# PKU-Alignment/SafeVLA

Hardware: AMD Instinct MI355X
Metric: env-steps/sec through PPO-Lagrangian update (higher is better)
Workload: dtype bf16

## Files before the change

### safevla_amd/csrc/attn.hip

```cpp
#include "common.h"
#include "attn_hd96.h"
#include "attn_long.h"

#ifndef ATT_SWZ_OLD
#define ATT_SWZ_OLD 0
#endif
#ifndef ATT_EARLY_TR
#define ATT_EARLY_TR 0
#endif
#define HD 64
#define LDSROW 64
#define ATT_THREADS 256

enum { MASK_NONE = 0, MASK_BLOCK_CAUSAL = 1 };

struct AttnArgs {
    const bf16_t *Q, *K, *V; long ld;
    bf16_t* O; long ldo;
    float* LSE;
    const bf16_t* dO; long lddo;
    bf16_t *dQ, *dK, *dV; long ldd;
    const int* traj;
    const float* bias;
    const unsigned char* kvalid;
    int S, H, mask_mode;
    float scale;
    int kv_rows;
    int Sq;
    long ldq, lddq;
    float* Dws;
    DropCfg drop;
    int xcd_rows;
};

__device__ __forceinline__ unsigned long long att_drop_row(const AttnArgs& p, int r, int h, int q) {
    return ((unsigned long long)((size_t)r * p.H + h) * p.S + q) * (unsigned long long)((p.S + 3) & ~3);
}
__device__ __forceinline__ bool att_keep1(const DropCfg& c, unsigned long long e) {
    const unsigned x = drop_bits(c.key, e >> 1);
    return ((e & 1) ? (x >> 16) : (x & 0xffffu)) >= c.thr;
}

__device__ __forceinline__ int att_swz(int row) {
    const int x = (row >> 1) & 7;
    return ATT_SWZ_OLD ? x : ((((x + ((x >> 2) << 1)) & 3) << 1) | (x >> 2));
}

struct RowBase { const bf16_t* lo; const bf16_t* hi; };
__device__ __forceinline__ RowBase att_row_base(const bf16_t* tile, int lane) {
    const int ql = lane & 15, g = lane >> 4, f = att_swz(ql);
    return RowBase{tile + ql * LDSROW + ((g ^ f) << 3), tile + ql * LDSROW + (((g + 4) ^ f) << 3)};
}
struct TrBase { const bf16_t* d[4]; };
__device__ __forceinline__ TrBase att_tr_base(const bf16_t* tile, int lane) {
    const int ql = lane & 15, g = lane >> 4;
    const int row = 4 * g + (ql >> 2), f = att_swz(row);
    TrBase t;
#pragma unroll
    for (int dt = 0; dt < 4; ++dt) t.d[dt] = tile + row * LDSROW + (((2 * dt + ((ql & 3) >> 1)) ^ f) << 3) + 4 * (ql & 1);
    return t;
}
__device__ __forceinline__ bf16x8 lds_row8i(const bf16_t* lane_base, int tile_row0) {
    return *(const bf16x8*)(lane_base + tile_row0 * LDSROW);
}
__device__ __forceinline__ bf16x8 lds_tr8i(const bf16_t* lane_base_dt, int rA, int rB) {
    const bf16x4 lo = lds_tr16_b64(lane_base_dt + rA * LDSROW);
    const bf16x4 hi = lds_tr16_b64(lane_base_dt + rB * LDSROW);
    return bf16x8{lo[0], lo[1], lo[2], lo[3], hi[0], hi[1], hi[2], hi[3]};
}
__device__ __forceinline__ bf16x8 pack8(const float (&v)[8]) {
    u32x4 w;
#pragma unroll
    for (int i = 0; i < 4; ++i) w[i] = pack_bf2(v[2 * i], v[2 * i + 1]);
    return __builtin_bit_cast(bf16x8, w);
}
#define LOG2E 1.4426950408889634f
#define LN2 0.6931471805599453f

template <int SP, int THREADS = ATT_THREADS>
__device__ __forceinline__ void stage_head(bf16_t* dst, const bf16_t* src, long ld, int S, int tid) {
    constexpr int IT = SP * 8 / THREADS;
    u32x4 w[IT];
#pragma unroll
    for (int i = 0; i < IT; ++i) {
        const int q = tid + i * THREADS;
        const int row = q >> 3, c = q & 7;
        w[i] = u32x4{0, 0, 0, 0};
        if (row < S) w[i] = *(const u32x4*)(src + (size_t)row * ld + c * 8);
    }
#pragma unroll
    for (int i = 0; i < IT; ++i) {
        const int q = tid + i * THREADS;
        *(u32x4*)(dst + (q >> 3) * LDSROW + (((q & 7) ^ att_swz(q >> 3)) << 3)) = w[i];
    }
}

__device__ __forceinline__ bool masked(const AttnArgs& p, int q, int key, const int* traj_s, const unsigned char* kv_s) {
    if (key >= p.S) return true;
    if (p.mask_mode == MASK_BLOCK_CAUSAL && (key > q || traj_s[key] != traj_s[q])) return true;
    if (kv_s && !kv_s[key]) return true;
    return false;
}

template <int NKT, bool GENERIC, int NW = 4, bool EXACT = false>
__device__ __forceinline__ void attn_fwd_kernel_body(AttnArgs p) {
    p.drop = drop_resolve(p.drop);
    extern __shared__ __attribute__((aligned(16))) char smem[];
    constexpr int SP = NKT * 16;
    bf16_t* Ks = (bf16_t*)smem;
    bf16_t* Vs = Ks + SP * LDSROW;
    int* traj_s = (int*)(Vs + SP * LDSROW);
    unsigned char* kv_s = (unsigned char*)(traj_s + SP);
    const int tid = threadIdx.x, lane = tid & 63, wid = tid >> 6;
    const int r = blockIdx.x / p.H, h = blockIdx.x % p.H;
    const size_t tok0 = (size_t)r * p.kv_rows, mtok0 = (size_t)r * p.S;
    const int S = p.S;
    stage_head<SP, NW * 64>(Ks, p.K + tok0 * p.ld + h * HD, p.ld, S, tid);
    stage_head<SP, NW * 64>(Vs, p.V + tok0 * p.ld + h * HD, p.ld, S, tid);
    for (int i = tid; i < SP; i += NW * 64) {
        traj_s[i] = (p.traj && i < S) ? p.traj[mtok0 + i] : -1;
        kv_s[i] = (p.kvalid && i < S) ? p.kvalid[mtok0 + i] : 1;
    }
    const int ql = lane & 15, g = lane >> 4;
    const int Sq = p.Sq;
    const size_t qtok0 = (size_t)r * Sq;
    const int nqt = (Sq + 15) / 16;
    constexpr int MAXQT = (NKT + NW - 1) / NW;
    bf16x8 qall[MAXQT][2];
#pragma unroll
    for (int t = 0; t < MAXQT; ++t) {
        const int q = (wid + NW * t) * 16 + ql;
        const bool ok = q < Sq;
        const bf16_t* qp = p.Q + (qtok0 + (ok ? q : 0)) * p.ldq + h * HD + 8 * g;
        qall[t][0] = ok ? *(const bf16x8*)qp : bf16x8{0, 0, 0, 0, 0, 0, 0, 0};
        qall[t][1] = ok ? *(const bf16x8*)(qp + 32) : bf16x8{0, 0, 0, 0, 0, 0, 0, 0};
    }
    __syncthreads();
    const unsigned char* kvp = p.kvalid ? kv_s : nullptr;
    const RowBase Krow = att_row_base(Ks, lane);
    const TrBase Vtr = att_tr_base(Vs, lane);
#pragma unroll
    for (int t = 0; t < MAXQT; ++t) {
        const int qt = wid + NW * t;
        if (qt >= nqt) break;
        const int q = qt * 16 + ql;
        const bf16x8 qf[2] = {qall[t][0], qall[t][1]};
        float sc[NKT][4];
        float mx = -INFINITY;
        const float sl2 = p.scale * LOG2E;
#pragma unroll
        for (int kt = 0; kt < NKT; ++kt) {
            f32x4 a = {0.f, 0.f, 0.f, 0.f};
            if (EXACT || kt * 16 < S) {
                a = mfma16(lds_row8i(Krow.lo, kt * 16), qf[0], a);
                a = mfma16(lds_row8i(Krow.hi, kt * 16), qf[1], a);
            }
            if constexpr (GENERIC) {
#pragma unroll
                for (int e = 0; e < 4; ++e) {
                    const int key = kt * 16 + 4 * g + e;
                    float s = a[e] * p.scale;
                    if (p.bias && q < Sq && key < S) s += p.bias[((size_t)h * S + q) * S + key];
                    s *= LOG2E;
                    if (masked(p, q < Sq ? q : 0, key, traj_s, kvp)) s = -INFINITY;
                    sc[kt][e] = s;
                    mx = fmaxf(mx, s);
                }
            } else {
                const bool tail = EXACT ? kt >= NKT - 2 : (kt + 1) * 16 > S;
#pragma unroll
                for (int e = 0; e < 4; ++e) {
                    float s = a[e] * sl2;
                    if (tail && kt * 16 + 4 * g + e >= S) s = -INFINITY;
                    sc[kt][e] = s;
                    mx = fmaxf(mx, s);
                }
            }
        }
        mx = fmaxf(mx, __shfl_xor(mx, 16, 64));
        mx = fmaxf(mx, __shfl_xor(mx, 32, 64));
        if (mx == -INFINITY) mx = 0.f;
        float lsum = 0.f;
#pragma unroll
        for (int kt = 0; kt < NKT; ++kt)
#pragma unroll
            for (int e = 0; e < 4; ++e) { sc[kt][e] = __builtin_amdgcn_exp2f(sc[kt][e] - mx); lsum += sc[kt][e]; }
        lsum += __shfl_xor(lsum, 16, 64);
        lsum += __shfl_xor(lsum, 32, 64);
        if (p.drop.thr) {
            const unsigned long long rb = att_drop_row(p, r, h, q < Sq ? q : 0);
#pragma unroll
            for (int kt = 0; kt < NKT; ++kt) {
                const unsigned keep = drop_keep4(p.drop, rb + kt * 16 + 4 * g);
#pragma unroll
                for (int e = 0; e < 4; ++e) if (!((keep >> e) & 1u)) sc[kt][e] = 0.f;
            }
        }
        f32x4 o[4];
#pragma unroll
        for (int dt = 0; dt < 4; ++dt) o[dt] = f32x4{0.f, 0.f, 0.f, 0.f};
#pragma unroll
        for (int u = 0; u < NKT / 2; ++u) {
            if (EXACT || u * 32 < S) {
                const float pv[8] = {sc[2 * u][0], sc[2 * u][1], sc[2 * u][2], sc[2 * u][3],
                                     sc[2 * u + 1][0], sc[2 * u + 1][1], sc[2 * u + 1][2], sc[2 * u + 1][3]};
                const bf16x8 pa = pack8(pv);
#pragma unroll
                for (int dt = 0; dt < 4; ++dt)
                    o[dt] = mfma16(lds_tr8i(Vtr.d[dt], 32 * u, 32 * u + 16), pa, o[dt]);
            }
        }
        const float inv = lsum > 0.f ? p.drop.scale / lsum : 0.f;
        if (q < Sq) {
#pragma unroll
            for (int dt = 0; dt < 4; ++dt) {
                const u32x2 w = {pack_bf2(o[dt][0] * inv, o[dt][1] * inv), pack_bf2(o[dt][2] * inv, o[dt][3] * inv)};
                *(u32x2*)(p.O + (qtok0 + q) * p.ldo + h * HD + dt * 16 + 4 * g) = w;
            }
        }
        if (p.LSE && g == 0 && q < Sq) p.LSE[((size_t)r * p.H + h) * Sq + q] = (mx + __log2f(lsum)) * LN2;
    }
}

__device__ __forceinline__ void att_xcd_item(const AttnArgs& p, int item, int nitems, int& r, int& h) {
    if (!p.xcd_rows) return;
    const int x = item & 7, j = item >> 3, nfull = (nitems / 64) * 8;
    if ((j >> 3) * 8 + x < nfull) { r = (j >> 3) * 8 + x; h = j & 7; }
}
struct AttDrop {
    unsigned a0;
    unsigned hb;
    bool wrap;
    unsigned long long p0;
};
__device__ __forceinline__ AttDrop att_drop_head(const AttnArgs& p, int r, int h) {
    AttDrop d;
    d.p0 = att_drop_row(p, r, h, 0) >> 1;
    d.a0 = (unsigned)d.p0 * 0x9E3779B1u;
    d.hb = ((unsigned)(d.p0 >> 32) * 0x85EBCA77u) ^ p.drop.key;
    d.wrap = (unsigned)d.p0 > 0xFFFF0000u;
    return d;
}

template <int NKT>
__device__ __forceinline__ void attn_fwd_persist_kernel_body(AttnArgs p, int nitems) {
    p.drop = drop_resolve(p.drop);
    extern __shared__ __attribute__((aligned(16))) char smem[];
    constexpr int SP = NKT * 16, IT = SP * 8 / ATT_THREADS, MAXQT = (NKT + 3) / 4;
    bf16_t* Ks = (bf16_t*)smem;
    bf16_t* Vs = Ks + SP * LDSROW;
    const int tid = threadIdx.x, lane = tid & 63, wid = tid >> 6;
    const int ql = lane & 15, g = lane >> 4;
    const int S = p.S, Sq = p.Sq, nqt = (Sq + 15) / 16;
    u32x4 kreg[IT], vreg[IT];
    bf16x8 qreg[MAXQT][2];
    auto fetch = [&](int item) {
        int r = item / p.H, h = item % p.H;
        att_xcd_item(p, item, nitems, r, h);
        const bf16_t* kp = p.K + (size_t)r * p.kv_rows * p.ld + h * HD;
        const bf16_t* vp = p.V + (size_t)r * p.kv_rows * p.ld + h * HD;
#pragma unroll
        for (int i = 0; i < IT; ++i) {
            const int q = tid + i * ATT_THREADS, row = q >> 3, c = q & 7;
            kreg[i] = u32x4{0, 0, 0, 0}; vreg[i] = u32x4{0, 0, 0, 0};
            if (row < S) {
                kreg[i] = *(const u32x4*)(kp + (size_t)row * p.ld + c * 8);
                vreg[i] = *(const u32x4*)(vp + (size_t)row * p.ld + c * 8);
            }
        }
#pragma unroll
        for (int t = 0; t < MAXQT; ++t) {
            const int q = (wid + 4 * t) * 16 + ql;
            const bool ok = q < Sq;
            const bf16_t* qp = p.Q + ((size_t)r * Sq + (ok ? q : 0)) * p.ldq + h * HD + 8 * g;
            qreg[t][0] = ok ? *(const bf16x8*)qp : bf16x8{0, 0, 0, 0, 0, 0, 0, 0};
            qreg[t][1] = ok ? *(const bf16x8*)(qp + 32) : bf16x8{0, 0, 0, 0, 0, 0, 0, 0};
        }
    };
    int item = blockIdx.x;
    if (item >= nitems) return;
    fetch(item);
    const RowBase Krow = att_row_base(Ks, lane);
    const TrBase Vtr = att_tr_base(Vs, lane);
    const float sl2 = p.scale * LOG2E;
    for (; item < nitems; item += gridDim.x) {
        int r = item / p.H, h = item % p.H;
        att_xcd_item(p, item, nitems, r, h);
        const size_t qtok0 = (size_t)r * Sq;
        __syncthreads();
#pragma unroll
        for (int i = 0; i < IT; ++i) {
            const int q = tid + i * ATT_THREADS;
            const int off = (q >> 3) * LDSROW + (((q & 7) ^ att_swz(q >> 3)) << 3);
            *(u32x4*)(Ks + off) = kreg[i];
            *(u32x4*)(Vs + off) = vreg[i];
        }
        bf16x8 qcur[MAXQT][2];
#pragma unroll
        for (int t = 0; t < MAXQT; ++t) { qcur[t][0] = qreg[t][0]; qcur[t][1] = qreg[t][1]; }
        __syncthreads();
        if (item + (int)gridDim.x < nitems) fetch(item + gridDim.x);
#pragma unroll
        for (int t = 0; t < MAXQT; ++t) {
            const int qt = wid + 4 * t;
// ... 508 lines not shown
#pragma unroll
                for (int dt = 0; dt < 4; ++dt) {
                    const u32x2 wk = {pack_bf2(dk[dt][0], dk[dt][1]), pack_bf2(dk[dt][2], dk[dt][3])};
                    const u32x2 wv = {pack_bf2(dv[dt][0], dv[dt][1]), pack_bf2(dv[dt][2], dv[dt][3])};
                    *(u32x2*)(p.dK + (tok0 + keyl) * p.ldd + h * HD + dt * 16 + 4 * g) = wk;
                    *(u32x2*)(p.dV + (tok0 + keyl) * p.ldd + h * HD + dt * 16 + 4 * g) = wv;
                }
            }
        }
    }
}

__device__ __forceinline__ f32x4 fma4(f32x4 a, f32x4 b, f32x4 c) { return __builtin_elementwise_fma(a, b, c); }

template <int NKT, bool DROP>
__global__ void __launch_bounds__(ATT_THREADS, NKT <= 12 ? 3 : 2) attn_bwd_fused_exact_kernel(AttnArgs p) {
    if (DROP) p.drop = drop_resolve(p.drop);
#ifdef ATT_TIMING
    const long long tm0 = __builtin_readcyclecounter();
#endif
    extern __shared__ __attribute__((aligned(16))) char smem[];
    constexpr int SP = NKT * 16, MAXT = (NKT + 3) / 4, IT = SP * 8 / ATT_THREADS;
    constexpr bool EARLY_TR = ATT_EARLY_TR && NKT <= 12;
    constexpr bool KEEP_KV = true;
    bf16_t* As = (bf16_t*)smem;
    bf16_t* Bs = As + SP * LDSROW;
    float* nl_s = (float*)(Bs + SP * LDSROW);
    float* nd_s = nl_s + SP;
    const int tid = threadIdx.x, lane = tid & 63, wid = tid >> 6;
    int r = blockIdx.x / p.H, h = blockIdx.x % p.H;
    att_xcd_item(p, blockIdx.x, gridDim.x, r, h);
    const size_t tok0 = (size_t)r * p.S, qtok0 = (size_t)r * p.Sq;
    const int S = p.S, Sq = p.Sq;
    const int ql = lane & 15, g = lane >> 4;
    constexpr int NBUF = KEEP_KV ? MAXT : 2;
    bf16x8 kvbuf[NBUF][4];
    auto load_kv = [&](int t, bf16x8 (&dst)[4]) {
        const int keyl = (wid + 4 * t) * 16 + ql;
        const bool kok = keyl < S;
        const bf16_t* kp = p.K + (tok0 + (kok ? keyl : 0)) * p.ld + h * HD + 8 * g;
        const bf16_t* vp = p.V + (tok0 + (kok ? keyl : 0)) * p.ld + h * HD + 8 * g;
        dst[0] = gld8(kp, kok); dst[1] = gld8(kp + 32, kok);
        dst[2] = gld8(vp, kok); dst[3] = gld8(vp + 32, kok);
    };
    load_kv(0, kvbuf[0]);
    if (KEEP_KV) {
#pragma unroll
        for (int t = 1; t < MAXT; ++t) if (wid + 4 * t < NKT) load_kv(t, kvbuf[t]);
    }
    stage_head<SP>(As, p.Q + qtok0 * p.ldq + h * HD, p.ldq, Sq, tid);
    {
        u32x4 w[IT];
        float part[IT];
#pragma unroll
        for (int i = 0; i < IT; ++i) {
            const int q = tid + i * ATT_THREADS, row = q >> 3, c = q & 7;
            const bool ok = row < Sq;
            const bf16x8 gv = gld8(p.dO + (qtok0 + (ok ? row : 0)) * p.lddo + h * HD + c * 8, ok);
            const bf16x8 ov = gld8(p.O + (qtok0 + (ok ? row : 0)) * p.ldo + h * HD + c * 8, ok);
            w[i] = __builtin_bit_cast(u32x4, gv);
            part[i] = dot8(gv, ov);
        }
#pragma unroll
        for (int i = 0; i < IT; ++i) {
            const int q = tid + i * ATT_THREADS, row = q >> 3;
            *(u32x4*)(Bs + row * LDSROW + (((q & 7) ^ att_swz(row)) << 3)) = w[i];
            float d = part[i];
            d += __shfl_xor(d, 1, 64); d += __shfl_xor(d, 2, 64); d += __shfl_xor(d, 4, 64);
            if ((q & 7) == 0) nd_s[row] = -d * p.scale;
        }
    }
    for (int i = tid; i < SP; i += ATT_THREADS)
        nl_s[i] = i < Sq ? -p.LSE[((size_t)r * p.H + h) * Sq + i] * LOG2E : -INFINITY;
    __syncthreads();
#ifdef ATT_TIMING
    const long long tm1 = __builtin_readcyclecounter();
#endif
    const float sl2 = p.scale * LOG2E;
    const float dsc = DROP ? p.drop.scale : 1.f, scd = p.scale * dsc;
    const f32x4 sl4 = {sl2, sl2, sl2, sl2}, scd4 = {scd, scd, scd, scd}, dsc4 = {dsc, dsc, dsc, dsc};
    const RowBase Arow = att_row_base(As, lane), Brow = att_row_base(Bs, lane);
    const TrBase Atr = att_tr_base(As, lane), Btr = att_tr_base(Bs, lane);
    const int S4 = (S + 3) & ~3, hS = S4 >> 1;
    AttDrop dh{};
    if (DROP) dh = att_drop_head(p, r, h);
    const unsigned thr = p.drop.thr;
    {
        const int nw = (Sq + 31) / 32;
        const int odd = ql & 1;
        const unsigned dl_a = (unsigned)((4 * g + 2 * odd) * hS + (ql >> 1));
        const unsigned al_a = dh.a0 + dl_a * 0x9E3779B1u;
        const unsigned hSC = (unsigned)hS * 0x9E3779B1u;
#pragma unroll
        for (int t = 0; t < MAXT; ++t) {
            const int kt = wid + 4 * t;
            __builtin_amdgcn_sched_barrier(0);
            if (kt < NKT) {
                const int keyl = kt * 16 + ql;
                const bool kok = keyl < S;
                if (!KEEP_KV && t + 1 < MAXT && kt + 4 < NKT) load_kv(t + 1, kvbuf[(t + 1) % NBUF]);
                const bf16x8 kf0 = kvbuf[t % NBUF][0], kf1 = kvbuf[t % NBUF][1], vf0 = kvbuf[t % NBUF][2], vf1 = kvbuf[t % NBUF][3];
                f32x4 dk[4], dv[4];
#pragma unroll
                for (int dt = 0; dt < 4; ++dt) { dk[dt] = f32x4{0.f, 0.f, 0.f, 0.f}; dv[dt] = f32x4{0.f, 0.f, 0.f, 0.f}; }
#pragma unroll (NKT <= 12 ? 2 : 1)
                for (int w = 0; w < nw; ++w) {
                    const int off = w * 32 * LDSROW;
                    float pv[8], dsv[8];
                    bf16x8 gfr[4], qfr[4];
                    if (EARLY_TR) {
#pragma unroll
                        for (int dt = 0; dt < 4; ++dt) { gfr[dt] = lds_tr8i(Btr.d[dt] + off, 0, 16); qfr[dt] = lds_tr8i(Atr.d[dt] + off, 0, 16); }
                    }
#pragma unroll
                    for (int e2 = 0; e2 < 2; ++e2) {
                        const int o2 = off + e2 * 16 * LDSROW;
                        f32x4 sv = {0.f, 0.f, 0.f, 0.f}, dp = {0.f, 0.f, 0.f, 0.f};
                        sv = mfma16(*(const bf16x8*)(Arow.lo + o2), kf0, sv);
                        sv = mfma16(*(const bf16x8*)(Arow.hi + o2), kf1, sv);
                        dp = mfma16(*(const bf16x8*)(Brow.lo + o2), vf0, dp);
                        dp = mfma16(*(const bf16x8*)(Brow.hi + o2), vf1, dp);
                        const f32x4 nl4 = *(const f32x4*)(nl_s + w * 32 + e2 * 16 + 4 * g), nd4 = *(const f32x4*)(nd_s + w * 32 + e2 * 16 + 4 * g);
                        const f32x4 x = fma4(sv, sl4, nl4);
                        f32x4 pr;
#pragma unroll
                        for (int e = 0; e < 4; ++e) pr[e] = __builtin_amdgcn_exp2f(x[e]);
                        f32x4 pd = pr, tt = fma4(dp, scd4, nd4);
                        if (DROP) {
                            pd = pr * dsc4;
                            unsigned keep;
                            if (!dh.wrap) {
                                const int qb = w * 32 + e2 * 16;
                                const unsigned ua = (unsigned)(qb * hS + kt * 8) * 0x9E3779B1u;
                                const unsigned x0 = drop_mix((al_a + ua) ^ dh.hb), x1 = drop_mix((al_a + ua + hSC) ^ dh.hb);
                                const unsigned mine = odd ? ((x0 >> 16) | (x1 & 0xffff0000u)) : ((x0 & 0xffffu) | (x1 << 16));
                                const unsigned give = odd ? ((x0 & 0xffffu) | (x1 << 16)) : ((x0 >> 16) | (x1 & 0xffff0000u));
                                const unsigned got = (unsigned)__builtin_amdgcn_mov_dpp((int)give, 0xB1, 0xf, 0xf, true);
                                const unsigned q01 = odd ? got : mine, q23 = odd ? mine : got;
                                keep = ((q01 & 0xffffu) >= thr ? 1u : 0u) | ((q01 >> 16) >= thr ? 2u : 0u) | ((q23 & 0xffffu) >= thr ? 4u : 0u) | ((q23 >> 16) >= thr ? 8u : 0u);
                            } else {
                                keep = 0;
#pragma unroll
                                for (int e = 0; e < 4; ++e) {
                                    const int q = w * 32 + e2 * 16 + 4 * g + e;
                                    keep |= att_keep1(p.drop, (dh.p0 << 1) + (unsigned)(q * S4 + keyl)) ? (1u << e) : 0u;
                                }
                            }
#pragma unroll
                            for (int e = 0; e < 4; ++e) {
                                const bool kp = (keep >> e) & 1u;
                                pd[e] = kp ? pd[e] : 0.f;
                                tt[e] = kp ? tt[e] : nd4[e];
                            }
                        }
                        const f32x4 ds = pr * tt;
#pragma unroll
                        for (int e = 0; e < 4; ++e) { pv[e2 * 4 + e] = pd[e]; dsv[e2 * 4 + e] = ds[e]; }
                    }
                    const bf16x8 pa = pack8(pv), da = pack8(dsv);
#pragma unroll
                    for (int dt = 0; dt < 4; ++dt) {
                        if (!EARLY_TR) { gfr[dt] = lds_tr8i(Btr.d[dt] + off, 0, 16); qfr[dt] = lds_tr8i(Atr.d[dt] + off, 0, 16); }
                        dv[dt] = mfma16(gfr[dt], pa, dv[dt]);
                        dk[dt] = mfma16(qfr[dt], da, dk[dt]);
                    }
                }
                if (kok) {
#pragma unroll
                    for (int dt = 0; dt < 4; ++dt) {
                        const u32x2 wk = {pack_bf2(dk[dt][0], dk[dt][1]), pack_bf2(dk[dt][2], dk[dt][3])};
                        const u32x2 wv = {pack_bf2(dv[dt][0], dv[dt][1]), pack_bf2(dv[dt][2], dv[dt][3])};
                        *(u32x2*)(p.dK + (tok0 + keyl) * p.ldd + h * HD + dt * 16 + 4 * g) = wk;
                        *(u32x2*)(p.dV + (tok0 + keyl) * p.ldd + h * HD + dt * 16 + 4 * g) = wv;
                    }
                }
            }
        }
    }
    __builtin_amdgcn_sched_barrier(0);
#ifdef ATT_TIMING
    const long long tm2 = __builtin_readcyclecounter();
#endif
    bf16x8 qall[MAXT][4];
    float dall[MAXT], lall[MAXT];
#pragma unroll
    for (int t = 0; t < MAXT; ++t) {
        const int qt = wid + 4 * t;
        if (qt < NKT) {
            const int o = qt * 16 * LDSROW;
            qall[t][0] = *(const bf16x8*)(Arow.lo + o); qall[t][1] = *(const bf16x8*)(Arow.hi + o);
            qall[t][2] = *(const bf16x8*)(Brow.lo + o); qall[t][3] = *(const bf16x8*)(Brow.hi + o);
            lall[t] = nl_s[qt * 16 + ql]; dall[t] = nd_s[qt * 16 + ql];
        }
    }
    __syncthreads();
    if (KEEP_KV) {
        const int f = att_swz(ql);
#pragma unroll
        for (int t = 0; t < MAXT; ++t) {
            const int kt = wid + 4 * t;
            if (kt < NKT) {
                bf16_t* ka = As + (kt * 16 + ql) * LDSROW;
                bf16_t* va = Bs + (kt * 16 + ql) * LDSROW;
                *(bf16x8*)(ka + ((g ^ f) << 3)) = kvbuf[t % NBUF][0]; *(bf16x8*)(ka + (((g + 4) ^ f) << 3)) = kvbuf[t % NBUF][1];
                *(bf16x8*)(va + ((g ^ f) << 3)) = kvbuf[t % NBUF][2]; *(bf16x8*)(va + (((g + 4) ^ f) << 3)) = kvbuf[t % NBUF][3];
            }
        }
    } else {
        stage_head<SP>(As, p.K + tok0 * p.ld + h * HD, p.ld, S, tid);
        stage_head<SP>(Bs, p.V + tok0 * p.ld + h * HD, p.ld, S, tid);
    }
    __syncthreads();
#ifdef ATT_TIMING
    const long long tm3 = __builtin_readcyclecounter();
#endif
    {
        const int ntile = (Sq + 15) / 16;
        const unsigned dl_b = (unsigned)(ql * hS + 2 * g);
        const unsigned al_b = dh.a0 + dl_b * 0x9E3779B1u;
#pragma unroll
        for (int t = 0; t < MAXT; ++t) {
            const int qt = wid + 4 * t;
            __builtin_amdgcn_sched_barrier(0);
            if (qt < ntile) {
                const int q = qt * 16 + ql;
                const bool qok = q < Sq;
                const f32x4 nl4 = {lall[t], lall[t], lall[t], lall[t]}, nd4 = {dall[t], dall[t], dall[t], dall[t]};
                f32x4 dq[4];
#pragma unroll
                for (int dt = 0; dt < 4; ++dt) dq[dt] = f32x4{0.f, 0.f, 0.f, 0.f};
#pragma unroll (NKT <= 12 ? 2 : 1)
                for (int u = 0; u < NKT / 2; ++u) {
                    const int off = u * 32 * LDSROW;
                    float dsv[8];
#pragma unroll
                    for (int e2 = 0; e2 < 2; ++e2) {
                        const int o2 = off + e2 * 16 * LDSROW;
                        f32x4 sv = {0.f, 0.f, 0.f, 0.f}, dp = {0.f, 0.f, 0.f, 0.f};
                        sv = mfma16(*(const bf16x8*)(Arow.lo + o2), qall[t][0], sv);
                        sv = mfma16(*(const bf16x8*)(Arow.hi + o2), qall[t][1], sv);
                        dp = mfma16(*(const bf16x8*)(Brow.lo + o2), qall[t][2], dp);
                        dp = mfma16(*(const bf16x8*)(Brow.hi + o2), qall[t][3], dp);
                        const f32x4 x = fma4(sv, sl4, nl4);
                        f32x4 pr;
#pragma unroll
                        for (int e = 0; e < 4; ++e) pr[e] = __builtin_amdgcn_exp2f(x[e]);
                        f32x4 tt = fma4(dp, scd4, nd4);
                        if (DROP) {
                            unsigned keep;
                            if (!dh.wrap) {
                                const unsigned ub = (unsigned)(qt * 16 * hS + (2 * u + e2) * 8) * 0x9E3779B1u;
                                const unsigned r0 = drop_mix((al_b + ub) ^ dh.hb), r1 = drop_mix((al_b + ub + 0x9E3779B1u) ^ dh.hb);
                                keep = ((r0 & 0xffffu) >= thr ? 1u : 0u) | ((r0 >> 16) >= thr ? 2u : 0u) | ((r1 & 0xffffu) >= thr ? 4u : 0u) | ((r1 >> 16) >= thr ? 8u : 0u);
                            } else {
                                keep = drop_keep4(p.drop, (dh.p0 << 1) + (unsigned long long)(qok ? q : 0) * S4 + (2 * u + e2) * 16 + 4 * g);
                            }
#pragma unroll
                            for (int e = 0; e < 4; ++e) tt[e] = ((keep >> e) & 1u) ? tt[e] : nd4[e];
                        }
                        const f32x4 ds = pr * tt;
#pragma unroll
                        for (int e = 0; e < 4; ++e) dsv[e2 * 4 + e] = ds[e];
                    }
                    const bf16x8 da = pack8(dsv);
#pragma unroll
                    for (int dt = 0; dt < 4; ++dt)
                        dq[dt] = mfma16(lds_tr8i(Atr.d[dt] + off, 0, 16), da, dq[dt]);
                }
                if (qok) {
#pragma unroll
                    for (int dt = 0; dt < 4; ++dt) {
                        const u32x2 w = {pack_bf2(dq[dt][0], dq[dt][1]), pack_bf2(dq[dt][2], dq[dt][3])};
                        *(u32x2*)(p.dQ + (qtok0 + q) * p.lddq + h * HD + dt * 16 + 4 * g) = w;
                    }
                }
            }
        }
    }
#ifdef ATT_TIMING
    if (p.kvalid && lane == 0) {
        __builtin_amdgcn_sched_barrier(0);
        const long long tm4 = __builtin_readcyclecounter();
        unsigned* d = (unsigned*)p.kvalid + ((size_t)blockIdx.x * 4 + wid) * 4;
        d[0] = (unsigned)(tm1 - tm0); d[1] = (unsigned)(tm2 - tm1); d[2] = (unsigned)(tm3 - tm2); d[3] = (unsigned)(tm4 - tm3);
    }
#endif
}

template <int NKT>
static int launch_fwd(const AttnArgs& p, int rows, hipStream_t st) {
    const size_t lds = (size_t)2 * NKT * 16 * LDSROW * sizeof(bf16_t) + NKT * 16 * (sizeof(int) + 1);
    const bool generic = p.mask_mode != MASK_NONE || p.bias || p.kvalid;
    if constexpr (NKT == 12 || NKT == 16) {
        if (!generic && p.S > (NKT - 2) * 16) {
            const size_t ldsp = (size_t)2 * NKT * 16 * LDSROW * sizeof(bf16_t);
            static int slots = 0;
            if (!slots) {
                int dev = 0, n_cu = 0;
                HIP_CHECK_RET(hipGetDevice(&dev));
                HIP_CHECK_RET(hipDeviceGetAttribute(&n_cu, hipDeviceAttributeMultiprocessorCount, dev));
                slots = 2 * n_cu;
            }
            const int nitems = rows * p.H;
            const int gslots = (slots / svla_group_size()) & ~7;
            return SVLA_LAUNCH_TWIN((attn_fwd_persist_kernel_body<NKT>), ATT_THREADS, 2, dim3(nitems < gslots ? nitems : gslots), dim3(ATT_THREADS), ldsp, st, p, nitems);
        }
    }
    if constexpr (NKT == 18) {
        if (!generic && p.S > (NKT - 2) * 16 && p.Sq == p.S)
            return SVLA_LAUNCH_TWIN((attn_fwd_kernel_body<NKT, false, 4, true>), ATT_THREADS, 1, dim3(rows * p.H), dim3(ATT_THREADS), lds, st, p);
    }
    if constexpr (NKT >= 28) {
        if (!generic) {
            if (p.S > (NKT - 2) * 16 && p.Sq == p.S) return SVLA_LAUNCH_TWIN((attn_fwd_kernel_body<NKT, false, 8, true>), 512, 1, dim3(rows * p.H), dim3(512), lds, st, p);
            return SVLA_LAUNCH_TWIN((attn_fwd_kernel_body<NKT, false, 8>), 512, 1, dim3(rows * p.H), dim3(512), lds, st, p);
        }
    }
    if (generic) return SVLA_LAUNCH_TWIN((attn_fwd_kernel_body<NKT, true>), ATT_THREADS, 1, dim3(rows * p.H), dim3(ATT_THREADS), lds, st, p);
    return SVLA_LAUNCH_TWIN((attn_fwd_kernel_body<NKT, false>), ATT_THREADS, 1, dim3(rows * p.H), dim3(ATT_THREADS), lds, st, p);
}
static int g_attn_no_decode = 0;
static int g_attn_bwd_two_pass = 0;
static int g_attn_xcd_rows = 1;
extern "C" int svla_attn_bwd_two_pass(int on) { g_attn_bwd_two_pass = on & 1; g_attn_xcd_rows = !(on & 2); g_attn_no_decode = (on & 4) ? 1 : 0; return 0; }

template <int NKT>
static int launch_bwd(const AttnArgs& p, int rows, hipStream_t st) {
    const size_t lds_q = (size_t)2 * NKT * 16 * LDSROW * sizeof(bf16_t) + NKT * 16 * (sizeof(int) + 1);
    const size_t lds_kv = (size_t)2 * NKT * 16 * LDSROW * sizeof(bf16_t) + NKT * 16 * (2 * sizeof(float) + sizeof(int) + 1);
    static bool attr = false;
    if (!attr) {
        HIP_CHECK_RET(hipFuncSetAttribute((const void*)attn_bwd_dq_kernel<NKT, true>, hipFuncAttributeMaxDynamicSharedMemorySize, (int)lds_q));
        HIP_CHECK_RET(hipFuncSetAttribute((const void*)attn_bwd_dkv_kernel<NKT, true>, hipFuncAttributeMaxDynamicSharedMemorySize, (int)lds_kv));
        HIP_CHECK_RET(hipFuncSetAttribute((const void*)attn_bwd_dq_kernel<NKT, false>, hipFuncAttributeMaxDynamicSharedMemorySize, (int)lds_q));
        HIP_CHECK_RET(hipFuncSetAttribute((const void*)attn_bwd_dkv_kernel<NKT, false>, hipFuncAttributeMaxDynamicSharedMemorySize, (int)lds_kv));
        attr = true;
    }
    const bool generic = p.mask_mode != MASK_NONE || p.bias || p.kvalid;
    if constexpr (NKT <= 16) if (!generic && (p.Dws || !g_attn_bwd_two_pass) && p.S > (NKT - 3) * 16) {
        const size_t le_q = (size_t)2 * NKT * 16 * LDSROW * sizeof(bf16_t);
        const size_t le_kv = le_q + NKT * 16 * 2 * sizeof(float);
        static bool attr_e = false;
        if (!attr_e) {
            HIP_CHECK_RET(hipFuncSetAttribute((const void*)attn_bwd_dq_exact_kernel<NKT>, hipFuncAttributeMaxDynamicSharedMemorySize, (int)le_q));
            HIP_CHECK_RET(hipFuncSetAttribute((const void*)attn_bwd_dkv_exact_kernel<NKT>, hipFuncAttributeMaxDynamicSharedMemorySize, (int)le_kv));
            HIP_CHECK_RET(hipFuncSetAttribute((const void*)attn_bwd_fused_exact_kernel<NKT, true>, hipFuncAttributeMaxDynamicSharedMemorySize, (int)le_kv));
            HIP_CHECK_RET(hipFuncSetAttribute((const void*)attn_bwd_fused_exact_kernel<NKT, false>, hipFuncAttributeMaxDynamicSharedMemorySize, (int)le_kv));
            attr_e = true;
        }
        if (g_attn_bwd_two_pass) {
            hipLaunchKernelGGL((attn_bwd_dq_exact_kernel<NKT>), dim3(rows * p.H), dim3(ATT_THREADS), le_q, st, p);
            hipLaunchKernelGGL((attn_bwd_dkv_exact_kernel<NKT>), dim3(rows * p.H), dim3(ATT_THREADS), le_kv, st, p);
        } else {
#ifdef ATT_TIMING
            AttnArgs pt = p; if (getenv("SVLA_ATTN_DBGBUF")) pt.kvalid = (const unsigned char*)strtoull(getenv("SVLA_ATTN_DBGBUF"), nullptr, 16);
            if (p.drop.thr) { hipLaunchKernelGGL((attn_bwd_fused_exact_kernel<NKT, true>), dim3(rows * p.H), dim3(ATT_THREADS), le_kv, st, pt); return svla_launch_status(); }
#endif
            if (p.drop.thr) hipLaunchKernelGGL((attn_bwd_fused_exact_kernel<NKT, true>), dim3(rows * p.H), dim3(ATT_THREADS), le_kv, st, p);
            else hipLaunchKernelGGL((attn_bwd_fused_exact_kernel<NKT, false>), dim3(rows * p.H), dim3(ATT_THREADS), le_kv, st, p);
        }
        return svla_launch_status();
    }
    if (generic) {
        hipLaunchKernelGGL((attn_bwd_dq_kernel<NKT, true>), dim3(rows * p.H), dim3(ATT_THREADS), lds_q, st, p);
        hipLaunchKernelGGL((attn_bwd_dkv_kernel<NKT, true>), dim3(rows * p.H), dim3(ATT_THREADS), lds_kv, st, p);
    } else {
        hipLaunchKernelGGL((attn_bwd_dq_kernel<NKT, false>), dim3(rows * p.H), dim3(ATT_THREADS), lds_q, st, p);
        hipLaunchKernelGGL((attn_bwd_dkv_kernel<NKT, false>), dim3(rows * p.H), dim3(ATT_THREADS), lds_kv, st, p);
    }
    return svla_launch_status();
}

#define DEC_THREADS 256
#define DEC_MAXB 16
__device__ __forceinline__ void attn_decode_kernel_body(AttnArgs p) {
    __shared__ float red[4][2];
    __shared__ float accs[4][64];
    const int tid = threadIdx.x, lane = tid & 63, wid = tid >> 6;
    const int g = tid >> 3, c = tid & 7;
    const int r = blockIdx.x / p.H, h = blockIdx.x % p.H;
    const int S = p.S;
    const size_t tok0 = (size_t)r * p.kv_rows;
    const unsigned char* kvr = p.kvalid ? p.kvalid + (size_t)r * S : nullptr;
    const float sl2 = p.scale * LOG2E;
    float qv[8];
    {
        const bf16x8 q8 = *(const bf16x8*)(p.Q + (size_t)r * p.ldq + h * HD + c * 8);
#pragma unroll
        for (int e = 0; e < 8; ++e) qv[e] = bf2f((bf16_t)q8[e]);
    }
    const int nb = (S + 31) >> 5;
    float sc[DEC_MAXB];
    unsigned vmask = 0;
    float mx = -INFINITY;
#pragma unroll
    for (int b = 0; b < DEC_MAXB; ++b) {
        sc[b] = -INFINITY;
        if (b < nb) {
            const int key = b * 32 + g;
            const bool ok = key < S && (!kvr || kvr[key]);
            if (ok) {
                const bf16x8 k8 = *(const bf16x8*)(p.K + (tok0 + key) * p.ld + h * HD + c * 8);
                float d = 0.f;
#pragma unroll
                for (int e = 0; e < 8; ++e) d = fmaf(qv[e], bf2f((bf16_t)k8[e]), d);
                sc[b] = d;
                vmask |= 1u << b;
            }
            float d = ok ? sc[b] : 0.f;
            d += __shfl_xor(d, 1, 64); d += __shfl_xor(d, 2, 64); d += __shfl_xor(d, 4, 64);
            sc[b] = ok ? d * sl2 : -INFINITY;
            mx = fmaxf(mx, sc[b]);
        }
    }
    mx = fmaxf(mx, __shfl_xor(mx, 8, 64)); mx = fmaxf(mx, __shfl_xor(mx, 16, 64)); mx = fmaxf(mx, __shfl_xor(mx, 32, 64));
    if (lane == 0) red[wid][0] = mx;
    __syncthreads();
    mx = fmaxf(fmaxf(red[0][0], red[1][0]), fmaxf(red[2][0], red[3][0]));
    if (mx == -INFINITY) mx = 0.f;
    float acc[8], lsum = 0.f;
#pragma unroll
    for (int e = 0; e < 8; ++e) acc[e] = 0.f;
#pragma unroll
    for (int b = 0; b < DEC_MAXB; ++b) {
        if (b < nb && ((vmask >> b) & 1u)) {
            const float pr = __builtin_amdgcn_exp2f(sc[b] - mx);
            lsum += pr;
            const float pb = bf2f(f2bf(pr));
            const bf16x8 v8 = *(const bf16x8*)(p.V + (tok0 + b * 32 + g) * p.ld + h * HD + c * 8);
#pragma unroll
            for (int e = 0; e < 8; ++e) acc[e] = fmaf(pb, bf2f((bf16_t)v8[e]), acc[e]);
        }
    }
    lsum += __shfl_xor(lsum, 1, 64); lsum += __shfl_xor(lsum, 2, 64); lsum += __shfl_xor(lsum, 4, 64);
    lsum += __shfl_xor(lsum, 8, 64); lsum += __shfl_xor(lsum, 16, 64); lsum += __shfl_xor(lsum, 32, 64);
#pragma unroll
    for (int e = 0; e < 8; ++e) {
        float a = acc[e];
        a += __shfl_xor(a, 8, 64); a += __shfl_xor(a, 16, 64); a += __shfl_xor(a, 32, 64);
        acc[e] = a;
    }
    if (lane == 0) red[wid][1] = lsum * 0.125f;
    if (lane < 8) {
#pragma unroll
        for (int e = 0; e < 8; ++e) accs[wid][lane * 8 + e] = acc[e];
    }
    __syncthreads();
    if (tid < 64) {
        const float ls = (red[0][1] + red[1][1]) + (red[2][1] + red[3][1]);
        const float o = (accs[0][tid] + accs[1][tid]) + (accs[2][tid] + accs[3][tid]);
        const float inv = ls > 0.f ? 1.f / ls : 0.f;
        p.O[(size_t)r * p.ldo + h * HD + tid] = f2bf(o * inv);
        if (p.LSE && tid == 0) p.LSE[(size_t)r * p.H + h] = (mx + __log2f(ls)) * LN2;
    }
}
__global__ void __launch_bounds__(DEC_THREADS) attn_decode_kernel(AttnArgs p) { attn_decode_kernel_body(p); }

extern "C" int svla_attn_fwd_bf16(const bf16_t* Q, const bf16_t* K, const bf16_t* V, long ld, bf16_t* O, long ldo, float* LSE,
                                  int rows, int S, int H, int head_dim, float scale, int mask_mode, const int* traj,
                                  const float* bias, const unsigned char* kvalid, int Sq, long ldq, int kv_rows, const svla_dropout* drop,
                                  void* stream) {
    if (head_dim == 96) return attn96_fwd_launch(Q, K, V, ld, O, ldo, LSE, rows, S, H, scale, mask_mode, traj, bias, kvalid, Sq, ldq, kv_rows, drop, stream);
    if (head_dim != HD || rows <= 0 || S <= 0 || S > 512 || (ld % 8) || H <= 0 || (kv_rows > 0 && kv_rows < S)) return SVLA_EINVAL;
    if (mask_mode == MASK_BLOCK_CAUSAL && !traj) return SVLA_EINVAL;
    if (Sq < 0 || Sq > S || (Sq > 0 && (ldq % 8))) return SVLA_EINVAL;
    AttnArgs p{};
    p.Q = Q; p.K = K; p.V = V; p.ld = ld; p.O = O; p.ldo = ldo; p.LSE = LSE; p.traj = traj; p.bias = bias; p.kvalid = kvalid;
    p.S = S; p.H = H; p.mask_mode = mask_mode; p.scale = scale;
    p.Sq = Sq > 0 ? Sq : S; p.ldq = Sq > 0 ? ldq : ld;
    p.kv_rows = kv_rows > 0 ? kv_rows : S;
    p.drop = drop_cfg(drop);
    p.xcd_rows = 0;
    hipStream_t st = (hipStream_t)stream;
    if (p.Sq == 1 && !bias && mask_mode == MASK_NONE && !p.drop.thr && !g_attn_no_decode) {
        SVLA_LAUNCH(attn_decode_kernel, attn_decode_kernel_body, DEC_THREADS, 1, dim3(rows * H), dim3(DEC_THREADS), 0, st, p);
        return svla_launch_status();
    }
    if (S <= 64) return launch_fwd<4>(p, rows, st);
    if (S <= 128) return launch_fwd<8>(p, rows, st);
    if (S <= 192) return launch_fwd<12>(p, rows, st);
    if (S <= 256) return launch_fwd<16>(p, rows, st);
    if (S <= 288) return launch_fwd<18>(p, rows, st);
    if (S <= 448) return launch_fwd<28>(p, rows, st);
    return launch_fwd<32>(p, rows, st);
}

extern "C" int svla_attn_bwd_bf16(const bf16_t* Q, const bf16_t* K, const bf16_t* V, long ld, const bf16_t* O, long ldo,
                                  const float* LSE, const bf16_t* dO, long lddo, bf16_t* dQ, bf16_t* dK, bf16_t* dV, long ldd,
                                  int rows, int S, int H, int head_dim, float scale, int mask_mode, const int* traj,
                                  const float* bias, const unsigned char* kvalid, int Sq, long ldq, long lddq, float* D_ws,
                                  const svla_dropout* drop, void* stream) {
    if (head_dim == 96)
        return attn96_bwd_launch(Q, K, V, ld, O, ldo, LSE, dO, lddo, dQ, dK, dV, ldd, rows, S, H, scale, mask_mode, traj, bias, kvalid, Sq, ldq, lddq, D_ws, drop, stream);
    if (head_dim == HD && S > 256)
        return attn_long_bwd_launch(Q, K, V, ld, O, ldo, LSE, dO, lddo, dQ, dK, dV, ldd, rows, S, H, scale, mask_mode, traj, bias, kvalid, Sq, ldq, lddq, D_ws, drop, stream);
    if (head_dim != HD || rows <= 0 || S <= 0 || S > 256 || (ld % 8) || (lddo % 8) || H <= 0) return SVLA_EINVAL;
    if (mask_mode == MASK_BLOCK_CAUSAL && !traj) return SVLA_EINVAL;
    if (Sq < 0 || Sq > S || (Sq > 0 && ((ldq % 8) || (lddq % 8)))) return SVLA_EINVAL;
    AttnArgs p{};
    p.Sq = Sq > 0 ? Sq : S; p.ldq = Sq > 0 ? ldq : ld; p.lddq = Sq > 0 ? lddq : ldd; p.kv_rows = S;
    p.Q = Q; p.K = K; p.V = V; p.ld = ld; p.O = (bf16_t*)O; p.ldo = ldo; p.LSE = (float*)LSE; p.dO = dO; p.lddo = lddo;
    p.dQ = dQ; p.dK = dK; p.dV = dV; p.ldd = ldd; p.traj = traj; p.bias = bias; p.kvalid = kvalid;
    p.S = S; p.H = H; p.mask_mode = mask_mode; p.scale = scale; p.Dws = D_ws; p.drop = drop_cfg(drop);
    p.xcd_rows = (g_attn_xcd_rows && H == 8) ? 1 : 0;
    hipStream_t st = (hipStream_t)stream;
    if (S <= 64) return launch_bwd<4>(p, rows, st);
    if (S <= 128) return launch_bwd<8>(p, rows, st);
    if (S <= 192) return launch_bwd<12>(p, rows, st);
    return launch_bwd<16>(p, rows, st);
}
```

Measured before the change: 7741.

## Add one-phase fused attention backward kernel for 12-tile sequences

Adds a new attention backward kernel for NKT=12 that keeps Q and dO resident in LDS and streams K/V tiles per wave. It computes dK and dV per key tile and accumulates dQ in registers across all tiles, with the D=rowsum(dO*O) precompute done in-kernel. The intent is to avoid the separate passes and extra LDS/global traffic of the existing fused exact backward. It also clamps the persistent forward grid slot count to at least 8 so small device groups never launch an empty grid. Register pressure from the dQ accumulators and the extra syncs per step may cost occupancy.

```diff
diff --git a/safevla_amd/csrc/attn.hip b/safevla_amd/csrc/attn.hip
--- a/safevla_amd/csrc/attn.hip
+++ b/safevla_amd/csrc/attn.hip
@@ -1,5 +1,6 @@
 #include "common.h"
 #include "attn_hd96.h"
+#include "attn_onephase.h"
 #include "attn_long.h"
 
 #ifndef ATT_SWZ_OLD
@@ -1114,7 +1115,7 @@
                 slots = 2 * n_cu;
             }
             const int nitems = rows * p.H;
-            const int gslots = (slots / svla_group_size()) & ~7;
+            const int gslots = max((slots / svla_group_size()) & ~7, 8);
             return SVLA_LAUNCH_TWIN((attn_fwd_persist_kernel_body<NKT>), ATT_THREADS, 2, dim3(nitems < gslots ? nitems : gslots), dim3(ATT_THREADS), ldsp, st, p, nitems);
         }
     }
@@ -1159,6 +1160,11 @@
             HIP_CHECK_RET(hipFuncSetAttribute((const void*)attn_bwd_fused_exact_kernel<NKT, true>, hipFuncAttributeMaxDynamicSharedMemorySize, (int)le_kv));
             HIP_CHECK_RET(hipFuncSetAttribute((const void*)attn_bwd_fused_exact_kernel<NKT, false>, hipFuncAttributeMaxDynamicSharedMemorySize, (int)le_kv));
             attr_e = true;
+        }
+        if constexpr (NKT == 12) {
+            if (!g_attn_bwd_two_pass && attn_onephase_wanted(rows, p.S, p.Sq, p.H))
+                return attn_onephase_bwd_launch(p.Q, p.K, p.V, p.ld, p.O, p.ldo, p.LSE, p.dO, p.lddo, p.dQ, p.dK, p.dV, p.ldd, rows, p.S, p.H, p.scale, p.ldq, p.lddq,
+                                                p.drop, p.xcd_rows, st);
         }
         if (g_attn_bwd_two_pass) {
             hipLaunchKernelGGL((attn_bwd_dq_exact_kernel<NKT>), dim3(rows * p.H), dim3(ATT_THREADS), le_q, st, p);
diff --git a/safevla_amd/csrc/attn_onephase.h b/safevla_amd/csrc/attn_onephase.h
--- /dev/null
+++ b/safevla_amd/csrc/attn_onephase.h
@@ -0,0 +1,7 @@
+#pragma once
+#include "common.h"
+
+bool attn_onephase_wanted(int rows, int S, int Sq, int H);
+int attn_onephase_bwd_launch(const bf16_t* Q, const bf16_t* K, const bf16_t* V, long ld, const bf16_t* O, long ldo, const float* LSE, const bf16_t* dO,
+                             long lddo, bf16_t* dQ, bf16_t* dK, bf16_t* dV, long ldd, int rows, int S, int H, float scale, long ldq, long lddq,
+                             const DropCfg& drop, int xcd_rows, hipStream_t stream);
diff --git a/safevla_amd/csrc/attn_onephase.hip b/safevla_amd/csrc/attn_onephase.hip
--- /dev/null
+++ b/safevla_amd/csrc/attn_onephase.hip
@@ -0,0 +1,282 @@
+#include "attn_onephase.h"
+#include <stdlib.h>
+
+#define OP_HD 64
+#define OP_ROW 64
+#define OP_NKT 12
+#define OP_SP (OP_NKT * 16)
+#define OP_THREADS 256
+#define OP_DSROW 32
+#define OP_DSBUF (64 * OP_DSROW)
+#define OP_LOG2E 1.4426950408889634f
+
+struct OnePhaseArgs {
+    const bf16_t *Q, *K, *V; long ld;
+    const bf16_t* O; long ldo;
+    const float* LSE;
+    const bf16_t* dO; long lddo;
+    bf16_t *dQ, *dK, *dV; long ldd;
+    int S, H;
+    float scale;
+    long ldq, lddq;
+    DropCfg drop;
+    int xcd_rows;
+};
+
+__device__ __forceinline__ int op_swz(int row) {
+    const int x = (row >> 1) & 7;
+    return (((x + ((x >> 2) << 1)) & 3) << 1) | (x >> 2);
+}
+struct OpRow { const bf16_t* lo; const bf16_t* hi; };
+__device__ __forceinline__ OpRow op_row_base(const bf16_t* img, int lane) {
+    const int ql = lane & 15, g = lane >> 4, f = op_swz(ql);
+    return OpRow{img + ql * OP_ROW + ((g ^ f) << 3), img + ql * OP_ROW + (((g + 4) ^ f) << 3)};
+}
+__device__ __forceinline__ const bf16_t* op_tr_base(const bf16_t* img, int lane, int dt) {
+    const int ql = lane & 15, g = lane >> 4;
+    const int row = 4 * g + (ql >> 2), f = op_swz(row);
+    return img + row * OP_ROW + (((2 * dt + ((ql & 3) >> 1)) ^ f) << 3) + 4 * (ql & 1);
+}
+template <int PITCH>
+__device__ __forceinline__ bf16x8 op_tr8(const bf16_t* lane_base) {
+    const bf16x4 lo = lds_tr16_b64(lane_base);
+    const bf16x4 hi = lds_tr16_b64(lane_base + 16 * PITCH);
+    return bf16x8{lo[0], lo[1], lo[2], lo[3], hi[0], hi[1], hi[2], hi[3]};
+}
+__device__ __forceinline__ bf16x8 op_gld8(const bf16_t* p, bool ok) { return ok ? *(const bf16x8*)p : bf16x8{0, 0, 0, 0, 0, 0, 0, 0}; }
+__device__ __forceinline__ float op_dot8(bf16x8 a, bf16x8 b) {
+    float s = 0.f;
+#pragma unroll
+    for (int i = 0; i < 8; ++i) s += bf2f((bf16_t)a[i]) * bf2f((bf16_t)b[i]);
+    return s;
+}
+__device__ __forceinline__ bf16x8 op_pack8(const float (&v)[8]) {
+    u32x4 w;
+#pragma unroll
+    for (int i = 0; i < 4; ++i) w[i] = pack_bf2(v[2 * i], v[2 * i + 1]);
+    return __builtin_bit_cast(bf16x8, w);
+}
+__device__ __forceinline__ f32x4 op_fma4(f32x4 a, f32x4 b, f32x4 c) { return __builtin_elementwise_fma(a, b, c); }
+
+template <bool DROP>
+__global__ void __launch_bounds__(OP_THREADS, 2) attn_bwd_onephase_kernel(OnePhaseArgs p) {
+    if (DROP) p.drop = drop_resolve(p.drop);
+    extern __shared__ __attribute__((aligned(16))) char smem[];
+    constexpr int SP = OP_SP, IT = SP * 8 / OP_THREADS;
+    bf16_t* Qs = (bf16_t*)smem;
+    bf16_t* Gs = Qs + SP * OP_ROW;
+    bf16_t* Kr = Gs + SP * OP_ROW;
+    bf16_t* Ds = Kr + 64 * OP_ROW;
+    float* nl_s = (float*)(Ds + 2 * OP_DSBUF);
+    float* nd_s = nl_s + SP;
+    const int tid = threadIdx.x, lane = tid & 63, wid = tid >> 6;
+    int r = blockIdx.x / p.H, h = blockIdx.x % p.H;
+    if (p.xcd_rows) {
+        const int item = blockIdx.x, x = item & 7, j = item >> 3, nfull = ((int)gridDim.x / 64) * 8;
+        if ((j >> 3) * 8 + x < nfull) { r = (j >> 3) * 8 + x; h = j & 7; }
+    }
+    const int S = p.S;
+    const size_t tok0 = (size_t)r * S;
+    const int ql = lane & 15, g = lane >> 4;
+    bf16x8 kvc[4], kvn[4];
+    auto load_kv = [&](int t, bf16x8 (&dst)[4]) {
+        const int keyl = (wid + 4 * t) * 16 + ql;
+        const bool kok = keyl < S;
+        const bf16_t* kp = p.K + (tok0 + (kok ? keyl : 0)) * p.ld + h * OP_HD + 8 * g;
+        const bf16_t* vp = p.V + (tok0 + (kok ? keyl : 0)) * p.ld + h * OP_HD + 8 * g;
+        dst[0] = op_gld8(kp, kok); dst[1] = op_gld8(kp + 32, kok);
+        dst[2] = op_gld8(vp, kok); dst[3] = op_gld8(vp + 32, kok);
+    };
+    load_kv(0, kvc);
+    {
+        u32x4 wq[IT], wg[IT];
+        float part[IT];
+#pragma unroll
+        for (int i = 0; i < IT; ++i) {
+            const int q = tid + i * OP_THREADS, row = q >> 3, c = q & 7;
+            const bool ok = row < S;
+            const bf16x8 qv = op_gld8(p.Q + (tok0 + (ok ? row : 0)) * p.ldq + h * OP_HD + c * 8, ok);
+            const bf16x8 gv = op_gld8(p.dO + (tok0 + (ok ? row : 0)) * p.lddo + h * OP_HD + c * 8, ok);
+            const bf16x8 ov = op_gld8(p.O + (tok0 + (ok ? row : 0)) * p.ldo + h * OP_HD + c * 8, ok);
+            wq[i] = __builtin_bit_cast(u32x4, qv);
+            wg[i] = __builtin_bit_cast(u32x4, gv);
+            part[i] = op_dot8(gv, ov);
+        }
+#pragma unroll
+        for (int i = 0; i < IT; ++i) {
+            const int q = tid + i * OP_THREADS, row = q >> 3;
+            const int o = row * OP_ROW + (((q & 7) ^ op_swz(row)) << 3);
+            *(u32x4*)(Qs + o) = wq[i];
+            *(u32x4*)(Gs + o) = wg[i];
+            float d = part[i];
+            d += __shfl_xor(d, 1, 64); d += __shfl_xor(d, 2, 64); d += __shfl_xor(d, 4, 64);
+            if ((q & 7) == 0) nd_s[row] = -d * p.scale;
+        }
+    }
+    for (int i = tid; i < SP; i += OP_THREADS)
+        nl_s[i] = i < S ? -p.LSE[((size_t)r * p.H + h) * S + i] * OP_LOG2E : -INFINITY;
+
+    const float sl2 = p.scale * OP_LOG2E;
+    const float dsc = DROP ? p.drop.scale : 1.f, scd = p.scale * dsc;
+    const f32x4 sl4 = {sl2, sl2, sl2, sl2}, scd4 = {scd, scd, scd, scd}, dsc4 = {dsc, dsc, dsc, dsc};
+    constexpr int GOFF = SP * OP_ROW;
+    const OpRow Qrow = op_row_base(Qs, lane);
+    const bf16_t* Qtr[4];
+#pragma unroll
+    for (int dt = 0; dt < 4; ++dt) Qtr[dt] = op_tr_base(Qs, lane, dt);
+    const bf16_t* Ktr = op_tr_base(Kr, lane, wid);
+    bf16_t* ds_st = Ds + (wid * 16 + ql) * OP_DSROW + 4 * g;
+    const int st_half = (ql >> 2) & 1;
+    const bf16_t* ds_ld = Ds + (4 * g + (ql >> 2)) * OP_DSROW + 4 * (ql & 3);
+    const int ld_half = g & 1;
+    const int S4 = (S + 3) & ~3, hS = S4 >> 1;
+    unsigned da0 = 0, dhb = 0;
+    if (DROP) {
+        const unsigned long long dp0 = (((unsigned long long)((size_t)r * p.H + h) * S) * (unsigned long long)S4) >> 1;
+        da0 = (unsigned)dp0 * 0x9E3779B1u;
+        dhb = ((unsigned)(dp0 >> 32) * 0x85EBCA77u) ^ p.drop.key;
+    }
+    const unsigned thr = p.drop.thr;
+    const int odd = ql & 1;
+    const unsigned al_a = da0 + (unsigned)((4 * g + 2 * odd) * hS + (ql >> 1)) * 0x9E3779B1u;
+    const unsigned hSC = (unsigned)hS * 0x9E3779B1u;
+
+    f32x4 dq[OP_NKT / 2][2];
+#pragma unroll
+    for (int w = 0; w < OP_NKT / 2; ++w) { dq[w][0] = f32x4{0.f, 0.f, 0.f, 0.f}; dq[w][1] = f32x4{0.f, 0.f, 0.f, 0.f}; }
+
+#pragma unroll 1
+    for (int t = 0; t < OP_NKT / 4; ++t) {
+        const int kt = wid + 4 * t;
+        const int keyl = kt * 16 + ql;
+        const bool kok = keyl < S;
+        {
+            const int f = op_swz(ql);
+            bf16_t* ka = Kr + (wid * 16 + ql) * OP_ROW;
+            *(bf16x8*)(ka + ((g ^ f) << 3)) = kvc[0];
+            *(bf16x8*)(ka + (((g + 4) ^ f) << 3)) = kvc[1];
+        }
+        __syncthreads();
+        const bf16x8 ka0 = op_tr8<OP_ROW>(Ktr), ka1 = op_tr8<OP_ROW>(Ktr + 32 * OP_ROW);
+        const bf16x8 kf0 = kvc[0], kf1 = kvc[1], vf0 = kvc[2], vf1 = kvc[3];
+        f32x4 dk[4], dv[4];
+#pragma unroll
+        for (int dt = 0; dt < 4; ++dt) { dk[dt] = f32x4{0.f, 0.f, 0.f, 0.f}; dv[dt] = f32x4{0.f, 0.f, 0.f, 0.f}; }
+#pragma unroll
+        for (int w = 0; w < OP_NKT / 2; ++w) {
+            const int off = w * 32 * OP_ROW;
+            float pv[8], dsv[8];
+            __builtin_amdgcn_sched_barrier(0);
+            if (w == OP_NKT / 2 - 2 && t + 1 < OP_NKT / 4) load_kv(t + 1, kvn);
+#pragma unroll
+            for (int e2 = 0; e2 < 2; ++e2) {
+                const int o2 = off + e2 * 16 * OP_ROW;
+                f32x4 sv = {0.f, 0.f, 0.f, 0.f}, dp = {0.f, 0.f, 0.f, 0.f};
+                sv = mfma16(*(const bf16x8*)(Qrow.lo + o2), kf0, sv);
+                sv = mfma16(*(const bf16x8*)(Qrow.hi + o2), kf1, sv);
+                dp = mfma16(*(const bf16x8*)(Qrow.lo + GOFF + o2), vf0, dp);
+                dp = mfma16(*(const bf16x8*)(Qrow.hi + GOFF + o2), vf1, dp);
+                const f32x4 nl4 = *(const f32x4*)(nl_s + w * 32 + e2 * 16 + 4 * g), nd4 = *(const f32x4*)(nd_s + w * 32 + e2 * 16 + 4 * g);
+                const f32x4 x = op_fma4(sv, sl4, nl4);
+                f32x4 pr;
+#pragma unroll
+                for (int e = 0; e < 4; ++e) pr[e] = __builtin_amdgcn_exp2f(x[e]);
+                f32x4 pd = pr, tt = op_fma4(dp, scd4, nd4);
+                if (DROP) {
+                    pd = pr * dsc4;
+                    unsigned keep;
+                    const int qb = w * 32 + e2 * 16;
+                    int hSw = __builtin_amdgcn_readfirstlane(hS);
+                    asm volatile("" : "+s"(hSw));
+                    const unsigned ua = (unsigned)(qb * hSw + kt * 8) * 0x9E3779B1u;
+                    const unsigned x0 = drop_mix((al_a + ua) ^ dhb), x1 = drop_mix((al_a + ua + hSC) ^ dhb);
+                    const unsigned mine = odd ? ((x0 >> 16) | (x1 & 0xffff0000u)) : ((x0 & 0xffffu) | (x1 << 16));
+                    const unsigned give = odd ? ((x0 & 0xffffu) | (x1 << 16)) : ((x0 >> 16) | (x1 & 0xffff0000u));
+                    const unsigned got = (unsigned)__builtin_amdgcn_mov_dpp((int)give, 0xB1, 0xf, 0xf, true);
+                    const unsigned q01 = odd ? got : mine, q23 = odd ? mine : got;
+                    keep = ((q01 & 0xffffu) >= thr ? 1u : 0u) | ((q01 >> 16) >= thr ? 2u : 0u) | ((q23 & 0xffffu) >= thr ? 4u : 0u) | ((q23 >> 16) >= thr ? 8u : 0u);
+#pragma unroll
+                    for (int e = 0; e < 4; ++e) {
+                        const bool kp = (keep >> e) & 1u;
+                        pd[e] = kp ? pd[e] : 0.f;
+                        tt[e] = kp ? tt[e] : nd4[e];
+                    }
+                }
+                const f32x4 ds = pr * tt;
+#pragma unroll
+                for (int e = 0; e < 4; ++e) { pv[e2 * 4 + e] = pd[e]; dsv[e2 * 4 + e] = ds[e]; }
+            }
+            const bf16x8 pa = op_pack8(pv), da = op_pack8(dsv);
+            {
+                const u32x4 dw = __builtin_bit_cast(u32x4, da);
+                bf16_t* st = ds_st + (w & 1) * OP_DSBUF;
+                *(u32x2*)(st + (st_half << 4)) = u32x2{dw[0], dw[1]};
+                *(u32x2*)(st + ((st_half ^ 1) << 4)) = u32x2{dw[2], dw[3]};
+            }
+#pragma unroll
+            for (int dt = 0; dt < 4; ++dt) {
+                dv[dt] = mfma16(op_tr8<OP_ROW>(Qtr[dt] + GOFF + off), pa, dv[dt]);
+                dk[dt] = mfma16(op_tr8<OP_ROW>(Qtr[dt] + off), da, dk[dt]);
+            }
+            __syncthreads();
+            const bf16_t* rd = ds_ld + (w & 1) * OP_DSBUF;
+#pragma unroll
+            for (int e2 = 0; e2 < 2; ++e2) {
+                const bf16_t* l2 = rd + ((e2 ^ ld_half) << 4);
+                dq[w][e2] = mfma16(ka0, op_tr8<OP_DSROW>(l2), dq[w][e2]);
+                dq[w][e2] = mfma16(ka1, op_tr8<OP_DSROW>(l2 + 32 * OP_DSROW), dq[w][e2]);
+            }
+        }
+        if (kok) {
+#pragma unroll
+            for (int dt = 0; dt < 4; ++dt) {
+                const u32x2 wk = {pack_bf2(dk[dt][0], dk[dt][1]), pack_bf2(dk[dt][2], dk[dt][3])};
+                const u32x2 wv = {pack_bf2(dv[dt][0], dv[dt][1]), pack_bf2(dv[dt][2], dv[dt][3])};
+                *(u32x2*)(p.dK + (tok0 + keyl) * p.ldd + h * OP_HD + dt * 16 + 4 * g) = wk;
+                *(u32x2*)(p.dV + (tok0 + keyl) * p.ldd + h * OP_HD + dt * 16 + 4 * g) = wv;
+            }
+        }
+#pragma unroll
+        for (int i = 0; i < 4; ++i) kvc[i] = kvn[i];
+    }
+#pragma unroll
+    for (int w = 0; w < OP_NKT / 2; ++w) {
+#pragma unroll
+        for (int e2 = 0; e2 < 2; ++e2) {
+            const int q = w * 32 + e2 * 16 + ql;
+            if (q < S) {
+                const f32x4 a = dq[w][e2];
+                *(u32x2*)(p.dQ + (tok0 + q) * p.lddq + h * OP_HD + wid * 16 + 4 * g) = u32x2{pack_bf2(a[0], a[1]), pack_bf2(a[2], a[3])};
+            }
+        }
+    }
+}
+
+static constexpr size_t OP_LDS = (size_t)(2 * OP_SP * OP_ROW + 64 * OP_ROW + 2 * OP_DSBUF) * sizeof(bf16_t) + (size_t)OP_SP * 2 * sizeof(float);
+
+bool attn_onephase_wanted(int rows, int S, int Sq, int H) {
+    if (S <= (OP_NKT - 2) * 16 || S > OP_SP || Sq != S) return false;
+    if ((unsigned long long)rows * H * S * ((S + 3) & ~3) / 2 > 0xFFFF0000ull) return false;
+    const char* e = getenv("SVLA_ATTN_ONEPHASE");
+    if (e && e[0] == '0') return false;
+    return true;
+}
+
+int attn_onephase_bwd_launch(const bf16_t* Q, const bf16_t* K, const bf16_t* V, long ld, const bf16_t* O, long ldo, const float* LSE, const bf16_t* dO,
+                             long lddo, bf16_t* dQ, bf16_t* dK, bf16_t* dV, long ldd, int rows, int S, int H, float scale, long ldq, long lddq,
+                             const DropCfg& drop, int xcd_rows, hipStream_t stream) {
+    if (S <= (OP_NKT - 2) * 16 || S > OP_SP || rows <= 0 || H <= 0) return SVLA_EINVAL;
+    static bool attr = false;
+    if (!attr) {
+        HIP_CHECK_RET(hipFuncSetAttribute((const void*)attn_bwd_onephase_kernel<true>, hipFuncAttributeMaxDynamicSharedMemorySize, (int)OP_LDS));
+        HIP_CHECK_RET(hipFuncSetAttribute((const void*)attn_bwd_onephase_kernel<false>, hipFuncAttributeMaxDynamicSharedMemorySize, (int)OP_LDS));
+        attr = true;
+    }
+    OnePhaseArgs p{};
+    p.Q = Q; p.K = K; p.V = V; p.ld = ld; p.O = O; p.ldo = ldo; p.LSE = LSE; p.dO = dO; p.lddo = lddo;
+    p.dQ = dQ; p.dK = dK; p.dV = dV; p.ldd = ldd; p.S = S; p.H = H; p.scale = scale; p.ldq = ldq; p.lddq = lddq;
+    p.drop = drop; p.xcd_rows = xcd_rows;
+    if (drop.thr) hipLaunchKernelGGL((attn_bwd_onephase_kernel<true>), dim3(rows * H), dim3(OP_THREADS), OP_LDS, stream, p);
+    else hipLaunchKernelGGL((attn_bwd_onephase_kernel<false>), dim3(rows * H), dim3(OP_THREADS), OP_LDS, stream, p);
+    return svla_launch_status();
+}
```

New measurement: 7809, median of 6. Within noise of the previous version (+0.9%).
